# msyriac/orphics

Hardware: AMD Instinct MI355X
Metric: QE kappa reconstructions/sec on 8192^2 maps (higher is better)
Workload: dtype f64

## Files before the change

### include/orphics_amd.h

```cpp
#ifndef ORPHICS_AMD_H
#define ORPHICS_AMD_H

#include <stddef.h>
#include <stdint.h>

#ifdef __cplusplus
extern "C" {
#endif

#define OA_F32 0
#define OA_F64 1

typedef struct oa_plan oa_plan;

const char* oa_last_error(void);
#define OA_ABI_VERSION 416
int oa_version(void);
int oa_device_count(void);

int oa_plan_create(int ny, int nx, int dtype, oa_plan** out);
int oa_plan_destroy(oa_plan* p);
long oa_plan_kpitch(const oa_plan* p);
long oa_plan_scratch_bytes(const oa_plan* p);
int oa_plan_set_laxes(oa_plan* p, const double* host_ly, const double* host_lx);
// ... 13 lines not shown
int oa_qe_map_legs_cols(oa_plan* p, const void* real_map, const void* FG, const void* FH, void* gx, void* gy, void* h,
                        int width, int rband, void* stream);
int oa_qe_cols_div(oa_plan* p, const void* px_rows, const void* py_rows, const void* Fnorm, void* out, int accumulate,
                   int width, int rband, void* stream);

int oa_plan_set_filters(oa_plan* p, const void* FG, const void* FH, const void* Fnorm, int leg_cols, int kappa_cols,
                        int leg_rows, int kappa_rows, int mrow);
int oa_plan_set_col_grid(oa_plan* p, int mcol);
int oa_plan_col_grid(const oa_plan* p);
int oa_plan_band_grid(const oa_plan* p, int* my, int* mx);
int oa_qe_band_bind(oa_plan* p, int nfilters, const void* const* host_filters, int nnorms, const void* const* host_Fnorm, int leg_cols,
                    int kappa_cols, int leg_rows, int kappa_rows, int mrow, int mcol, int max_leg_planes);
int oa_qe_band_grid(const oa_plan* p, int* my, int* mx);
int oa_plan_rsplit(const oa_plan* p);
int oa_plan_div_fused(const oa_plan* p);
enum { OA_OPT_MC_BATCH = 1, OA_OPT_MV_BATCH = 2, OA_OPT_MV_ROWBATCH = 3, OA_OPT_MV_CHAIN = 4, OA_OPT_DIV_BIN = 5, OA_OPT_WIN_FUSED = 6, OA_OPT_DRAW_FUSED = 7 };
int oa_plan_set_option(oa_plan* p, int option, int value);
int oa_plan_set_bins(oa_plan* p, const int32_t* ids_hc, int nids, double norm, void* stream);
void* oa_plan_kappa(oa_plan* p);
const int64_t* oa_plan_bin_counts(oa_plan* p);
int oa_qe_tt(oa_plan* p, const void* real_map, const void* kX, const void* kY, void* out_kappa_hc, int zero_outside,
             void* stream);
int oa_qe_pol(oa_plan* p, int npieces, const double* host_signs, const void* const* host_FG, const void* const* host_FH,
              const int* host_swap, const void* kX, const void* kY, const void* Fnorm, void* out, int accumulate,
              int leg_cols, int kappa_cols, int leg_rows, int kappa_rows, int mrow, int zero_outside, void* stream);
int oa_qe_mv(oa_plan* p, int nest, const int* host_npieces, const double* host_signs, const void* const* host_FG,
             const void* const* host_FH, const int* host_swap, const void* const* host_kX, const void* const* host_kY,
             const void* const* host_Fnorm, void* out, int accumulate, int leg_cols, int kappa_cols, int leg_rows, int kappa_rows,
             int mrow, int zero_outside, void* stream);
int oa_qe_mv_maps(oa_plan* p, int nmaps, const void* const* host_maps, const void* rot_c, const void* rot_s, int nest,
                  const int* host_npieces, const double* host_signs, const void* const* host_FG, const void* const* host_FH,
// ... 135 lines not shown
```

### orphics_amd/csrc/common.hpp

```cpp
#pragma once
#include <hip/hip_runtime.h>
#include <cstdio>
#include <cstring>
#include <string>
#include "../../include/orphics_amd.h"
#include "cx.hpp"

namespace oa {

std::string& last_error_ref();

inline int fail(const std::string& msg) {
    last_error_ref() = msg;
    return 1;
}

#define OA_HIP(expr)                                                                              \
    do {                                                                                          \
        hipError_t _e = (expr);                                                                   \
        if (_e != hipSuccess)                                                                     \
            return ::oa::fail(std::string(#expr) + ": " + hipGetErrorString(_e) + " (" + __FILE__ + \
                              ":" + std::to_string(__LINE__) + ")");                              \
    } while (0)

// ... 49 lines not shown
    double* ly64;
    double* lx64;
    bool have_laxes;
    bool pow2;
    oa_plan* inner;
    int My, Mx;
    void* chirp_y; void* chirp_x;
    void* cz_bhat; void* cz_a; void* cz_f;
    void* cz_full;
    bool mixed;
    void* mr_twx; void* mr_twxh; void* mr_twy;
    void* pipe;
    void* rq8c[5];
    void* tw_y_small[16];
    void* tw_y_m3[16];
};

namespace oa {
int plan_ensure_scratch(oa_plan* p, size_t bytes);
int czt_setup(oa_plan* p);
void czt_release(oa_plan* p);
int czt_c2c(oa_plan* p, const void* in, void* out, int inverse, double scale, hipStream_t st);
int czt_r2c(oa_plan* p, const void* real_in, void* hc_out, double scale, hipStream_t st);
int czt_c2r(oa_plan* p, const void* hc_in, void* real_out, double scale, hipStream_t st);
bool mixed_sides_ok(int ny, int nx);
int mixed_setup(oa_plan* p);
void mixed_release(oa_plan* p);
int mixed_c2c(oa_plan* p, const void* in, void* out, int inverse, double scale, hipStream_t st);
int mixed_r2c(oa_plan* p, const void* real_in, void* hc_out, double scale, hipStream_t st);
int mixed_c2r(oa_plan* p, const void* hc_in, void* real_out, double scale, hipStream_t st);
// ... 105 lines not shown
```

### orphics_amd/csrc/fft.hip

```cpp
#include <algorithm>
#include <cmath>
#include <vector>
#include "fft_launch.hpp"
#include "fft_r2c_w64.hpp"
#include "fft_r2c_rs4096.hpp"
#include "fft_divbin.hpp"

namespace oa {

template <typename T, int MODE, class SEQ>
__global__ __launch_bounds__(row_maxnt<SEQ>(), waves_per_eu<T>()) void row_fft_kernel(RowArgs<T> a) {
    GpuCtx c{oa_dyn_smem};
    row_fft_body<T, MODE, SEQ>(c, a);
}

#ifndef OA_W64_OCC
#define OA_W64_OCC 1
#endif
__global__ __launch_bounds__(64, OA_W64_OCC) void row_r2c_w64_kernel(RowW64Args a) {
    GpuCtx c{oa_dyn_smem};
    row_r2c_w64_body(c, a);
}

template <typename T, class SEQ, int LR, bool PF>
// ... 33 lines not shown
__global__ __launch_bounds__((sizeof(T) == 8 ? 512 : 1024)) void col_fband_pack_kernel(ColFBandArgs<T> a, cx<T>* out) {
    GpuCtx c{nullptr};
    col_fband_pack_body<T, SEQF, LR, LOGC>(c, a, out);
}
template <typename T, class SEQF, int LR, int LOGC>
__global__ __launch_bounds__((sizeof(T) == 8 ? 512 : 1024), (sizeof(T) == 8 ? 2 : 4)) void col_fband_kernel(ColFBandArgs<T> a) {
    GpuCtx c{oa_dyn_smem};
    col_fband_body<T, SEQF, LR, LOGC>(c, a);
}

template <typename T, class SEQF, int LOGC>
__global__ __launch_bounds__((sizeof(T) == 8 ? 512 : 1024)) void col_fband3_pack_kernel(ColFBandArgs<T> a, cx<T>* out) {
    GpuCtx c{nullptr};
    col_fband3_pack_body<T, SEQF, LOGC>(c, a, out);
}
template <typename T, class SEQF, int LOGC>
__global__ __launch_bounds__((sizeof(T) == 8 ? 512 : 1024), (sizeof(T) == 8 ? 2 : 4)) void col_fband3_kernel(ColFBandArgs<T> a) {
    GpuCtx c{oa_dyn_smem};
    col_fband3_body<T, SEQF, LOGC>(c, a);
}

__global__ __launch_bounds__(128, 1) void row_r2c_w64x2_kernel(RowW64Args a) {
    GpuCtx c{oa_dyn_smem};
    row_r2c_w64x2_body(c, a);
}

#ifndef OA_QE_WAVES_PER_EU
#define OA_QE_WAVES_PER_EU 3
#endif
template <typename T, class SEQ> constexpr int qe_waves_per_eu() {
    return sizeof(T) == 8 ? 1 : (row_maxnt<SEQ>() > 256 ? 2 : OA_QE_WAVES_PER_EU);
}

template <typename T, class SEQ, int NZ>
// ... 274 lines not shown
    void col_fband_pack(int gx, int gy, int logMy, const ColFBandArgs<T>& a, cx<T>* out) {
        if (rc) return;
        const int lt = Fft2dPlan<T>::fband_lt(), nt = (1 << lt) / EPT;
        const bool narrow = lt < (sizeof(T) == 4 ? 14 : 13);
        const bool ok = dispatch_fband<T>(gy, logMy, narrow, [&](auto seq, auto lrc, auto lcc) {
            hipLaunchKernelGGL((col_fband_pack_kernel<T, decltype(seq), decltype(lrc)::value, decltype(lcc)::value>), dim3(gx, gy), dim3(nt), 0, st, a, out);
            const hipError_t e = hipGetLastError();
            if (e != hipSuccess) rc = fail(std::string("fft launch: ") + hipGetErrorString(e));
        });
        if (!ok) rc = fail("fft: unsupported R-split column stage");
    }
    template <typename T>
    void col_fband3(int gx, int gz, size_t smem, int logMy, const ColFBandArgs<T>& a) {
        if (rc) return;
        constexpr int nt = sizeof(T) == 4 ? 1024 : 512, lc11 = sizeof(T) == 4 ? 3 : 2;
        if (logMy == 11) go(col_fband3_kernel<T, Seq<16, 16, 8>, lc11>, dim3(gx, 4, gz), nt, smem, a);
        else if (logMy == 10) go(col_fband3_kernel<T, Seq<16, 8, 8>, lc11 + 1>, dim3(gx, 4, gz), nt, smem, a);
        else rc = fail("fft: unsupported 3 x 2^k R-split column stage");
    }
    template <typename T>
    void col_fband3_pack(int gx, int logMy, const ColFBandArgs<T>& a, cx<T>* out) {
        if (rc) return;
        constexpr int nt = sizeof(T) == 4 ? 1024 : 512, lc11 = sizeof(T) == 4 ? 3 : 2;
        if (logMy == 11) hipLaunchKernelGGL((col_fband3_pack_kernel<T, Seq<16, 16, 8>, lc11>), dim3(gx, 4), dim3(nt), 0, st, a, out);
        else if (logMy == 10) hipLaunchKernelGGL((col_fband3_pack_kernel<T, Seq<16, 8, 8>, lc11 + 1>), dim3(gx, 4), dim3(nt), 0, st, a, out);
        else { rc = fail("fft: unsupported 3 x 2^k R-split column stage"); return; }
        const hipError_t e = hipGetLastError();
        if (e != hipSuccess) rc = fail(std::string("fft launch: ") + hipGetErrorString(e));
    }
    template <typename T>
    void row_qe(int grid, int nt, size_t smem, const RowQeArgs<T>& a) {
        const bool ok = dispatch_seq_qe(a.logL, [&](auto seq) {
            using S = decltype(seq);
// ... 329 lines not shown
    const size_t plane = (size_t)p->ny * p->kp * sizeof(cx<T>);
    if (int rc = plan_ensure_scratch(p, 2 * plane)) return rc;
    HipLauncher q{st};
    auto f = view<T>(p);
    cx<T>* tA = (cx<T>*)p->scratch;
    cx<T>* tB = tA + (size_t)p->ny * p->kp;
    const int w = f.clampw(width);
    const long pw = pwork > 0 ? pwork : p->kp;
    if (lr > 0) {
        const auto cv = coarse_view<T>(p, my);
        if (is_m3(my)) {
            const int myf = m3_pow2(my);
            const long kplane3 = (long)myf * pw;
            if (stages & 1) f.rows_rsplit(q, map, tA, pw, kplane3, w, myf);
            if (stages & 4) f.legs_fband3(q, cv, (const cx<T>*)p->tw_y_small[ilog2(myf)], tA, kplane3, pw, (const T*)FG, (const T*)FH, (const T*)p->lxd,
                                          (const T*)p->lyd, (cx<T>*)gx, (cx<T>*)gy, (cx<T>*)h, width, rband, pout > 0 ? pout : p->kp, 1, 0, 0, (const cx<T>*)fgh);
            return q.rc;
        }
        const long kplane = (long)my * pw;
        if (stages & 1) f.rows_rsplit(q, map, tA, pw, kplane, w, my);
        if (stages & 4) f.legs_fband(q, cv, tA, kplane, pw, (const T*)FG, (const T*)FH, (const T*)p->lxd, (const T*)p->lyd, (cx<T>*)gx, (cx<T>*)gy,
                                     (cx<T>*)h, width, rband, pout > 0 ? pout : p->kp, 1, 0, 0, (const cx<T>*)fgh);
        return q.rc;
    }
    if (stages & 1) f.rows(q, ROW_R2C, map, p->nx / 2, tA, pw, (T)1, w);
    if (my > 0 && my < p->ny) {
        if (stages & 2) f.cols(q, tA, pw, tB, pw, w, false, (T)1, 1);
        if (stages & 4) {
            static const bool nofuse = exp_env("OA_NO_FWDLEGS_CG") != nullptr;
            const auto cv = coarse_view<T>(p, my);
            if (nofuse || !f.legs_cols_from_pass1_cg(q, cv, tB, (const T*)FG, (const T*)FH, (const T*)p->lxd, (const T*)p->lyd,
// ... 66 lines not shown
    const long ms = (long)p->ny * pl, cms = (long)my * pl, gms = (long)my * pk;
    if (2 * ms > (long)p->ny * p->kp || 2 * gms > (long)p->ny * p->kp) return -1;
    const size_t plane = (size_t)p->ny * p->kp * sizeof(cx<T>);
    if (int rc = plan_ensure_scratch(p, 2 * plane)) return rc;
    HipLauncher q{st};
    q.fuse = fuse;
    cx<T>* tA = (cx<T>*)p->scratch;
    cx<T>* tB = tA + (size_t)p->ny * p->kp;
    const double s = 1.0 / ((double)p->ny * p->nx), sy = (double)p->ny / my;
    if (lr) {
        const int myf = m3 ? m3_pow2(my) : my;
        const long kplane = (long)myf * pl;
        f.rows_rsplit(q, map0, tA, pl, kplane, wi, myf);
        f.rows_rsplit(q, map1, tA + ms, pl, kplane, wi, myf);
        if (m3) f.legs_fband3(q, cv, (const cx<T>*)p->tw_y_small[ilog2(myf)], tA, kplane, pl, (const T*)FG, (const T*)FH, (const T*)p->lxd, (const T*)p->lyd,
                              (cx<T>*)c0, (cx<T>*)c1, (cx<T>*)c2, wl, rl, pl, 2, ms, cms, (const cx<T>*)fgh);
        else
        f.legs_fband(q, cv, tA, kplane, pl, (const T*)FG, (const T*)FH, (const T*)p->lxd, (const T*)p->lyd, (cx<T>*)c0, (cx<T>*)c1, (cx<T>*)c2, wl, rl,
                     pl, 2, ms, cms, (const cx<T>*)fgh);
        cv.rows_qe(q, (const cx<T>*)c0, (const cx<T>*)c1, (const cx<T>*)c2, (cx<T>*)g0, (cx<T>*)g1, (T)(s * s * sy), 0, wi, wo, mrow, pl, pk, 2, cms, gms,
                   -1, nullptr, lr);
        if (m3) cv.cols_div3(q, (const cx<T>*)g0, (const cx<T>*)g1, (const T*)Fn, (const T*)p->lxd, (const T*)p->lyd, (cx<T>*)out0, 0, wk, rk, pk, 2, gms,
                             (long)((cx<T>*)out1 - (cx<T>*)out0));
        else
        cv.cols_div(q, (const cx<T>*)g0, (const cx<T>*)g1, (const T*)Fn, (const T*)p->lxd, (const T*)p->lyd, (cx<T>*)out0, tA, tB, 0, wk, rk, pk, 2,
                    gms, gms, (long)((cx<T>*)out1 - (cx<T>*)out0));
        return q.rc;
    }
    f.rows(q, ROW_R2C, map0, p->nx / 2, tA, pl, (T)1, wi);
    f.rows(q, ROW_R2C, map1, p->nx / 2, tA + ms, pl, (T)1, wi);
    const cx<T>* ins[2] = {tA, tA + ms};
// ... 419 lines not shown
```

### orphics_amd/csrc/fft_fband.hpp

```cpp
#pragma once
#include "fft_kernels.hpp"
#include "fft_mixed.hpp"
#ifndef FB_STAMP
#define FB_STAMP(i)
#endif

namespace oa {

template <typename T>
struct ColFBandArgs {
    const cx<T>* in;
    long kplane, pitch;
    const T* FG; const T* FH;
    long fpitch;
    const cx<T>* fgh;
    const T* lxd; const T* lyd;
    cx<T>* gx; cx<T>* gy; cx<T>* h;
    long opitch;
    int width;
    const cx<T>* tw;
    int ny_full, rband;
    long in_moff, out_moff;
    const cx<T>* tw3 = nullptr;
};

template <typename T>
struct FBandStore2 {
    cx<T>* base;
    unsigned kstride;
    int ncols;
    const cx<T>* twl;
    int h, k1;
    template <typename U> OA_HD void put(int k, int c, cx<U> v) const {
        if (c >= ncols) return;
        if (k1) v = v * tw_lds(twl, h, k);
        base[(unsigned)k * kstride + (unsigned)c] = swp(v);
    }
};
// ... 158 lines not shown
    template <typename U> OA_HD void put(int k, int c, cx<U> v) const {
        if (c >= ncols) return;
        const int y = 3 * k + q;
        base[(unsigned)y * kstride + (unsigned)c] = swp(v * ti[y]);
    }
};

template <int Q>
OA_HD int fband3_bin(int m, int e) {
    constexpr int Ns = 2 * Q, RL = 8;
    if (e == 0) return m;
    if (e == 2) return m + Q + (RL - 1) * Ns;
    return 2 * m >= Q ? m + (RL - 1) * Ns : m + Q;
}

template <typename T, class SEQF, int LOGC, class Ctx>
OA_HD void col_fband3_body(Ctx& ctx, const ColFBandArgs<T>& a) {
    cx<T>* s = reinterpret_cast<cx<T>*>(ctx.smem());
    constexpr int logL = seq_total_log<SEQF>();
    constexpr int R = 4;
    constexpr int RL = SEQF::get(SEQF::n - 1), NB = EPT / RL;
    static_assert(RL == 8 && NB == 2, "col_fband3: the last forward radix is 8");
    constexpr int logQ = logL - 4, Q = 1 << logQ, Mq = 3 * Q;
    constexpr int C = 1 << LOGC;
    constexpr int NT = (1 << (logL + LOGC)) / EPT;
    constexpr int NTS = (Q << LOGC) / EPT;
    const int tid = ctx.tid();
    int tile = ctx.bid_x();
    if ((sizeof(cx<T>) << LOGC) < 128) {
        constexpr int G = 128 / (int)(sizeof(cx<T>) << LOGC), GW = 8 * G;
        const int nt = ctx.grid_x(), base = tile & ~(GW - 1), r = tile & (GW - 1);
        if (base + GW <= nt) tile = base + G * (r & 7) + (r >> 3);
    }
    const int c0 = tile << LOGC;
    const int k1 = ctx.bid_y();
    int ncols = a.width - c0;
    if (ncols > C) ncols = C;
    cx<T> gv[EPT];
    cx<T>* twl = s + (1 << (logL + LOGC));
    cx<T>* twq = twl + tw_lds_size(logL);
    cx<T>* ti = twq + tw_lds_size(logQ);
    FB_STAMP(0);
    tw_lds_fill<T>(ctx, twl, a.tw, logL, logL, NT);
    tw_lds_fill<T>(ctx, twq, a.tw, logL, logQ, NT);
    for (int i = tid; i < Mq; i += NT) ti[i] = a.tw3[(unsigned)k1 * (unsigned)i];
    ctx.sync();
    FB_STAMP(1);
    const long zmap = ctx.bid_z();
    const int c = tid & (C - 1), m = tid >> LOGC;
    const bool ok = c < ncols;
    T fgv[3], fhv[3], lyv[3];
    bool lv[3];
    const cx<T>* fq = a.fgh ? a.fgh + (((long)k1 * ctx.grid_x() + tile) * 3) * NT + tid : nullptr;
    const T lx = ldg(a.lxd + (ok ? c0 + c : 0));
    const cx<T> wq1 = ldg(a.tw3 + 4 * m), wq2 = ldg(a.tw3 + 8 * m);
#pragma unroll
    for (int e = 0; e < 3; ++e) {
        const int yf = k1 + R * fband3_bin<Q>(m, e);
        bool live = ok;
        if (a.rband) live = ok && !(yf >= a.rband && yf <= a.ny_full - a.rband);
        if (fq) {
            const cx<T> f = ldg(fq + e * NT);
            fgv[e] = f.x; fhv[e] = f.y;
        } else {
            const long fi = live ? (long)yf * a.fpitch + (c0 + c) : 0;
            fgv[e] = ldg(a.FG + fi);
            fhv[e] = ldg(a.FH + fi);
        }
        lyv[e] = ldg(a.lyd + (live ? yf : 0));
        lv[e] = live;
    }
    FB_STAMP(2);
    const ColLoad<T> ld{a.in + zmap * a.in_moff + (long)k1 * a.kplane + c0, (unsigned)a.pitch, ncols, false};
    col_pipeline_to_regs<T, SEQF>(ctx, s, gv, tid, NT, LOGC, twl, logL, ld);
    ctx.sync();
    FB_STAMP(3);
    cx<T> zh[3], zx[3], zy[3];
    const cx<T> xm = (2 * m >= Q) ? gv[RL - 1] : gv[RL];
#pragma unroll
    for (int e = 0; e < 3; ++e) {
        const cx<T> x = e == 0 ? gv[0] : (e == 2 ? gv[2 * RL - 1] : xm);
        const T fg = lv[e] ? fgv[e] : (T)0, fh = lv[e] ? fhv[e] : (T)0, ly = lv[e] ? lyv[e] : (T)0;
        const cx<T> g = mul_pi(x * fg);
        zh[e] = swp(x * fh);
        zx[e] = swp(g * (ok ? lx : (T)0));
        zy[e] = swp(g * ly);
    }
    MrDft<T, 3>::run(zh); MrDft<T, 3>::run(zx); MrDft<T, 3>::run(zy);
#pragma unroll
    for (int q = 0; q < 3; ++q) {
        const int at = ((q * Q + m) << LOGC) + c;
        cx<T> h = zh[q], x = zx[q], y = zy[q];
        if (q == 1) { h = h * wq1; x = x * wq1; y = y * wq1; }
        if (q == 2) { h = h * wq2; x = x * wq2; y = y * wq2; }
        s[at] = h;
        s[(Mq << LOGC) + at] = x;
        s[2 * (Mq << LOGC) + at] = y;
    }
    ctx.sync();
    FB_STAMP(4);
    const int sid = tid / NTS, tq = tid - sid * NTS;
    const int leg = sid / 3, q = sid - 3 * leg;
    cx<T>* outp = leg == 0 ? a.h : (leg == 1 ? a.gx : a.gy);
    using SI = typename SeqOf<logQ>::type;
    const FBand3Store<T> st{outp + zmap * a.out_moff + (long)k1 * a.opitch + c0, (unsigned)(R * a.opitch), leg < 3 ? ncols : 0, ti, q};
    fft_pipeline<T, false, false, true, SI>(ctx, s + sid * (Q << LOGC), tq, NTS, logQ, LOGC, 0, twq, logQ, NoLoad{}, st);
    FB_STAMP(5);
}

template <typename T, class SEQF, int LOGC, class Ctx>
OA_HD void col_fband3_pack_body(Ctx& ctx, const ColFBandArgs<T>& a, cx<T>* out) {
    constexpr int logL = seq_total_log<SEQF>(), R = 4, Q = 1 << (logL - 4), C = 1 << LOGC;
    constexpr int NT = (1 << (logL + LOGC)) / EPT;
    const int tid = ctx.tid(), tile = ctx.bid_x(), k1 = ctx.bid_y(), c0 = tile << LOGC;
    const int c = tid & (C - 1), m = tid >> LOGC;
    cx<T>* o = out + (((long)k1 * ctx.grid_x() + tile) * 3) * NT + tid;
#pragma unroll
    for (int e = 0; e < 3; ++e) {
        const int yf = k1 + R * fband3_bin<Q>(m, e);
        bool live = c0 + c < a.width;
        if (a.rband) live = live && !(yf >= a.rband && yf <= a.ny_full - a.rband);
        cx<T> f = mk<T>((T)0, (T)0);
// ... 7 lines not shown
```

### orphics_amd/csrc/fft_plan.hpp

```cpp
#pragma once
#include <cmath>
#include <cstdlib>
#include <vector>
#include "fft_kernels.hpp"
#include "fft_fband.hpp"
#include "fft_rowqe8.hpp"

namespace oa {

template <typename T>
inline std::vector<cx<T>> make_twiddles(int M) {
    std::vector<cx<T>> t((size_t)M);
    const long double tau = 6.283185307179586476925286766559005768L;
    for (int k = 0; k < M; ++k) {
        long double a = tau * (long double)k / (long double)M;
        t[(size_t)k].x = (T)cosl(a);
        t[(size_t)k].y = (T)(-sinl(a));
    }
    return t;
}

inline long kpitch_for(int nx) { return nx / 2 + 16; }

inline bool is_pow2(int v) { return v > 0 && (v & (v - 1)) == 0; }
inline bool is_m3(int v) { return v >= 3 && v % 3 == 0 && is_pow2(v / 3); }
inline int m3_pow2(int v) { return v / 3 * 4; }

template <typename T>
struct Fft2dPlan {
    int ny = 0, nx = 0, logNy = 0, logNx = 0;
    long kp = 0;
    const cx<T>* tw_x = nullptr;
    const cx<T>* tw_y = nullptr;
    const cx<T>* rq8c[RQ8_NGRIDS] = {};
    bool rq8_ready(int m) const { const int i = rq8_slot(m); return rowqe8_on() && i >= 0 && rq8c[i] != nullptr; }
    int ny_full = 0;
    int yshift() const { return ny_full > ny ? ny_full - ny : 0; }
    static constexpr int COLC = COL_LOGC;

    long work_pitch(int w) const {
        const long c = 1L << COLC;
// ... 67 lines not shown
        a.in = Y; a.kplane = kplane; a.pitch = pin; a.FG = FG; a.FH = FH; a.fpitch = kp; a.lxd = lxd; a.lyd = lyd; a.fgh = fgh;
        a.gx = gx; a.gy = gy; a.h = h; a.opitch = pout; a.width = clampw(wmax); a.tw = cv.tw_y; a.ny_full = ny; a.rband = clampr(rband);
        a.in_moff = in_moff; a.out_moff = out_moff;
        const int lt = fband_lt(), lc = lt - cv.logNy, Cs = 1 << lc;
        const int logMq = cv.logNy - (logNy - cv.logNy);
        const size_t smem = ((size_t)(1 << lt) + tw_lds_size(cv.logNy) + tw_lds_size(logMq) + (logNy - cv.logNy == 1 ? 0 : (1 << logMq))) * sizeof(cx<T>);
        if (pack_out) q.col_fband_pack((a.width + Cs - 1) / Cs, 1 << (logNy - cv.logNy), cv.logNy, a, pack_out);
        else q.col_fband((a.width + Cs - 1) / Cs, 1 << (logNy - cv.logNy), nmaps, smem, cv.logNy, a);
    }
    static bool has_rsplit3(int logNy, int logNx, int my3, int wl) {
        if (!is_m3(my3)) return false;
        const int myf = m3_pow2(my3);
        return (myf == 1024 || myf == 2048) && logNy - ilog2(myf) == 2 && has_rsplit(logNy, logNx, myf, wl) && fband_lt() == (sizeof(T) == 4 ? 14 : 13) &&
               div_lt() == fband_lt();
    }
    template <class Launcher>
    void legs_fband3(Launcher& q, const Fft2dPlan<T>& cv, const cx<T>* twf, const cx<T>* Y, long kplane, long pin, const T* FG, const T* FH,
                     const T* lxd, const T* lyd, cx<T>* gx, cx<T>* gy, cx<T>* h, int wmax, int rband, long pout, int nmaps = 1, long in_moff = 0,
                     long out_moff = 0, const cx<T>* fgh = nullptr, cx<T>* pack_out = nullptr) const {
        ColFBandArgs<T> a{};
        a.in = Y; a.kplane = kplane; a.pitch = pin; a.FG = FG; a.FH = FH; a.fpitch = kp; a.lxd = lxd; a.lyd = lyd; a.fgh = fgh;
        a.gx = gx; a.gy = gy; a.h = h; a.opitch = pout; a.width = clampw(wmax); a.tw = twf; a.tw3 = cv.tw_y; a.ny_full = ny; a.rband = clampr(rband);
        a.in_moff = in_moff; a.out_moff = out_moff;
        const int logMy = logNy - 2, lt = fband_lt(), lc = lt - logMy, Cs = 1 << lc, logQ = logMy - 4;
        const size_t smem = ((size_t)(1 << lt) + tw_lds_size(logMy) + tw_lds_size(logQ) + 3 * (1 << logQ)) * sizeof(cx<T>);
        if (pack_out) q.col_fband3_pack((a.width + Cs - 1) / Cs, logMy, a, pack_out);
        else q.col_fband3((a.width + Cs - 1) / Cs, nmaps, smem, logMy, a);
    }
    long fband_table_entries(const Fft2dPlan<T>& cv, int wmax) const {
        const int lc = fband_lt() - cv.logNy, Cs = 1 << lc;
        return (long)((clampw(wmax) + Cs - 1) / Cs) * Cs * cv.ny;
    }
    long fband3_table_entries(const Fft2dPlan<T>& cv, int wmax) const {
        const int lc = fband_lt() - (logNy - 2), Cs = 1 << lc;
        return (long)((clampw(wmax) + Cs - 1) / Cs) * Cs * cv.ny;
    }

    double row_grid_scale(int mrow) const { return (mrow > 0 && mrow < nx) ? (double)nx / (double)mrow : 1.0; }
    bool rows_qe_is_pair(int win, int wout, int mrow) const {
        if (mrow <= 0 || ny % 2) return false;
// ... 343 lines not shown
```

### orphics_amd/csrc/pipeline.hip

```cpp
#include <dlfcn.h>
#include <cstdlib>
#include <algorithm>
#include <functional>
#include <string>
#include <utility>
#include <vector>
#include "common.hpp"
#include "fft_plan.hpp"
#include "divbin_runs.hpp"

namespace oa {

constexpr int MC_BATCH_MAX = 6;

struct DevBuf {
    void* p = nullptr;
    size_t bytes = 0;
    int reserve(size_t need, bool zero = false) {
        if (bytes >= need) return 0;
        if (p) { OA_HIP(hipDeviceSynchronize()); release(); }
        OA_HIP(hipMalloc(&p, need));
        bytes = need;
        if (zero) OA_HIP(hipMemset(p, 0, need));
        return 0;
// ... 52 lines not shown
    DivTabs& tabs_of(int rows) { return (my3 && rows == my3) ? dt[1] : dt[0]; }
    const DivTabs& tabs_of(int rows) const { return (my3 && rows == my3) ? dt[1] : dt[0]; }
    unsigned long bind_gen = 1;
    DevBuf fb_t;
    unsigned long fb_gen = 0;
    int fb_my = 0, fb_wl = 0, fb_rl = 0;
    void** mv_ftab = nullptr;
    std::vector<const void*> mv_fkey;
    int opt_mc_batch = MC_BATCH_MAX;
    bool opt_mv_batch = true;
    bool opt_mv_rowbatch = true;
    bool opt_mv_chain = true;
    bool opt_divbin = true;
    bool opt_win_fused = true;
    bool opt_win_fused_set = false;
    int opt_draw_fused = -1;
    oa_plan* band = nullptr;
    int bmy = 0, bmx = 0;
    DevBuf bplanes;
    DevBuf bids;
    DevBuf brows;
    DevBuf bwin;
    DevBuf bsplit;
    int bs_cap = 0;
    DevBuf bs_tab;
    std::vector<const void*> bs_key;
    struct PolBind {
        bool bound = false;
        unsigned long gen = 0;
        oa_plan* plan = nullptr;
// ... 188 lines not shown

int oa_plan_set_option(oa_plan* p, int option, int value) {
    OA_REQUIRE(p, "oa_plan_set_option: NULL plan");
    Pipeline* q = pipe_of(p);
    switch (option) {
        case OA_OPT_MC_BATCH:
            OA_REQUIRE(value >= 0 && value <= MC_BATCH_MAX, "oa_plan_set_option: OA_OPT_MC_BATCH takes 0 (default) .. 6");
            q->opt_mc_batch = value ? value : MC_BATCH_MAX; return 0;
        case OA_OPT_MV_BATCH: q->opt_mv_batch = value != 0; return 0;
        case OA_OPT_MV_ROWBATCH: q->opt_mv_rowbatch = value != 0; return 0;
        case OA_OPT_MV_CHAIN: q->opt_mv_chain = value != 0; return 0;
        case OA_OPT_DIV_BIN: q->opt_divbin = value != 0; return 0;
        case OA_OPT_WIN_FUSED:
            q->opt_win_fused = value != 0; q->opt_win_fused_set = value >= 0; return 0;
        case OA_OPT_DRAW_FUSED: q->opt_draw_fused = value < 0 ? -1 : (value != 0); return 0;
        default: return fail("oa_plan_set_option: unknown option");
    }
}
}
namespace oa {
static void band_options(Pipeline* q) {
    for (oa_plan* inner : {q->band, q->pb.plan}) {
        if (!inner || !inner->pipe) continue;
        Pipeline* b = (Pipeline*)inner->pipe;
        b->opt_mc_batch = q->opt_mc_batch; b->opt_mv_batch = q->opt_mv_batch; b->opt_mv_rowbatch = q->opt_mv_rowbatch;
        b->opt_mv_chain = q->opt_mv_chain; b->opt_divbin = q->opt_divbin; b->opt_win_fused = q->opt_win_fused;
    }
}
}
extern "C" {
int oa_plan_rdn0_batched(const oa_plan* p) { return (p && p->pipe) ? ((const Pipeline*)p->pipe)->rdn0_ran_batched : 0; }
int oa_plan_rsplit(const oa_plan* p) {
    if (!p || !p->pipe) return 0;
    const Pipeline* q = (const Pipeline*)p->pipe;
    return q->FG ? (1 << qe_rsplit_lr(p, q->map_grid(), q->wl, q->wk, q->mrow)) & ~1 : 0;
}

int oa_plan_div_fused(const oa_plan* p) {
    if (!p || !p->pipe) return 0;
    const Pipeline* q = (const Pipeline*)p->pipe;
    if (p->mixed) { band_options((Pipeline*)q); return (q->FG && q->ids && q->band) ? oa_plan_div_fused(q->band) : 0; }
// ... 2171 lines not shown
```

### orphics_amd/engine.py

```python
import ctypes

import numpy as np
import torch

from . import _lib
from ._lib import OA_F32, OA_F64, check


def _ptr(t):
    return ctypes.c_void_p(t.data_ptr()) if t is not None else None


def _stream():
    return ctypes.c_void_p(torch.cuda.current_stream().cuda_stream)


def _dirty(t):
    mark_dirty(t)
    return t


_RDT = {"f32": torch.float32, "f64": torch.float64}
_CDT = {"f32": torch.complex64, "f64": torch.complex128}
_CODE = {"f32": OA_F32, "f64": OA_F64}
# ... 399 lines not shown
        n = self._same(a, b)
        if a.dtype != self.rdt or b.dtype != self.rdt:
            raise ValueError("axpby: dtype mismatch")
        out = torch.empty_like(a) if out is None else self._out(out, a, self.rdt, "axpby")
        check(self.lib.oa_axpby_real(self.code, _ptr(a), _ptr(b), _ptr(out), float(alpha), float(beta), n, _stream()))
        return out

    def rot2(self, c, s, i1, i2):
        n = self._same(c, s, i1, i2)
        if c.dtype != self.rdt or i1.dtype != self.cdt or i2.dtype != self.cdt or s.dtype != self.rdt:
            raise ValueError("rot2: dtype mismatch")
        o1, o2 = torch.empty_like(i1), torch.empty_like(i2)
        check(self.lib.oa_rot2(self.code, _ptr(c), _ptr(s), _ptr(i1), _ptr(i2), _ptr(o1), _ptr(o2), n, _stream()))
        return o1, o2

    OPTIONS = {"mc_batch": 1, "mv_batch": 2, "mv_rowbatch": 3, "mv_chain": 4, "div_bin": 5, "win_fused": 6, "draw_fused": 7}

    def set_option(self, name, value):
        if name not in self.OPTIONS:
            raise ValueError("unknown plan option %r (one of %s)" % (name, sorted(self.OPTIONS)))
        check(self.lib.oa_plan_set_option(self.plan, self.OPTIONS[name], int(value)))
        self._options = dict(getattr(self, "_options", {}), **{name: int(value)})

    def copy_options_to(self, other):
        for name, value in getattr(self, "_options", {}).items():
            other.set_option(name, value)

    def band_grid(self, leg_cols, kappa_cols, leg_rows, kappa_rows, mrow=-1, mcol=-1):
        if not self.mixed:
            return None
        return band_grid(self.ny, self.nx, leg_cols, kappa_cols, leg_rows, kappa_rows, mrow, mcol)
# ... 273 lines not shown
```

Baseline: 6074.

## Process multiple k-planes per workgroup in fband3 column kernel with prefetch

Templates the 3x2^k R-split column-band kernel on KPW, so one workgroup handles 1, 2 or 4 of the four residue planes in a loop. Twiddle tables are loaded once per workgroup, and the next plane's input taps and filters are prefetched while the current plane's FFT stages run. This amortizes setup and hides global-load latency, at the cost of fewer workgroups, more registers and more LDS for twiddles. The default KPW is 2 only for f32 with at least two maps, so this f64 workload keeps KPW=1 and runs only the restructured single-plane body.

```diff
diff --git a/include/orphics_amd.h b/include/orphics_amd.h
--- a/include/orphics_amd.h
+++ b/include/orphics_amd.h
@@ -51,7 +51,8 @@
 int oa_qe_band_grid(const oa_plan* p, int* my, int* mx);
 int oa_plan_rsplit(const oa_plan* p);
 int oa_plan_div_fused(const oa_plan* p);
-enum { OA_OPT_MC_BATCH = 1, OA_OPT_MV_BATCH = 2, OA_OPT_MV_ROWBATCH = 3, OA_OPT_MV_CHAIN = 4, OA_OPT_DIV_BIN = 5, OA_OPT_WIN_FUSED = 6, OA_OPT_DRAW_FUSED = 7 };
+enum { OA_OPT_MC_BATCH = 1, OA_OPT_MV_BATCH = 2, OA_OPT_MV_ROWBATCH = 3, OA_OPT_MV_CHAIN = 4, OA_OPT_DIV_BIN = 5, OA_OPT_WIN_FUSED = 6, OA_OPT_DRAW_FUSED = 7,
+       OA_OPT_FBAND3_KPW = 8 };
 int oa_plan_set_option(oa_plan* p, int option, int value);
 int oa_plan_set_bins(oa_plan* p, const int32_t* ids_hc, int nids, double norm, void* stream);
 void* oa_plan_kappa(oa_plan* p);
diff --git a/orphics_amd/csrc/common.hpp b/orphics_amd/csrc/common.hpp
--- a/orphics_amd/csrc/common.hpp
+++ b/orphics_amd/csrc/common.hpp
@@ -87,6 +87,7 @@
     void* rq8c[5];
     void* tw_y_small[16];
     void* tw_y_m3[16];
+    int fband3_kpw;
 };
 
 namespace oa {
diff --git a/orphics_amd/csrc/fft.hip b/orphics_amd/csrc/fft.hip
--- a/orphics_amd/csrc/fft.hip
+++ b/orphics_amd/csrc/fft.hip
@@ -71,10 +71,10 @@
     GpuCtx c{nullptr};
     col_fband3_pack_body<T, SEQF, LOGC>(c, a, out);
 }
-template <typename T, class SEQF, int LOGC>
+template <typename T, class SEQF, int LOGC, int KPW>
 __global__ __launch_bounds__((sizeof(T) == 8 ? 512 : 1024), (sizeof(T) == 8 ? 2 : 4)) void col_fband3_kernel(ColFBandArgs<T> a) {
     GpuCtx c{oa_dyn_smem};
-    col_fband3_body<T, SEQF, LOGC>(c, a);
+    col_fband3_body<T, SEQF, LOGC, KPW>(c, a);
 }
 
 __global__ __launch_bounds__(128, 1) void row_r2c_w64x2_kernel(RowW64Args a) {
@@ -379,9 +379,16 @@
     void col_fband3(int gx, int gz, size_t smem, int logMy, const ColFBandArgs<T>& a) {
         if (rc) return;
         constexpr int nt = sizeof(T) == 4 ? 1024 : 512, lc11 = sizeof(T) == 4 ? 3 : 2;
-        if (logMy == 11) go(col_fband3_kernel<T, Seq<16, 16, 8>, lc11>, dim3(gx, 4, gz), nt, smem, a);
-        else if (logMy == 10) go(col_fband3_kernel<T, Seq<16, 8, 8>, lc11 + 1>, dim3(gx, 4, gz), nt, smem, a);
-        else rc = fail("fft: unsupported 3 x 2^k R-split column stage");
+        auto launch = [&](auto kc) {
+            constexpr int KPW = decltype(kc)::value;
+            if (logMy == 11) go(col_fband3_kernel<T, Seq<16, 16, 8>, lc11, KPW>, dim3(gx, 4 / KPW, gz), nt, smem, a);
+            else if (logMy == 10) go(col_fband3_kernel<T, Seq<16, 8, 8>, lc11 + 1, KPW>, dim3(gx, 4 / KPW, gz), nt, smem, a);
+            else rc = fail("fft: unsupported 3 x 2^k R-split column stage");
+        };
+        if (a.kpw == 1) launch(std::integral_constant<int, 1>{});
+        else if (a.kpw == 2 || (a.kpw == 4 && sizeof(T) == 4)) launch(std::integral_constant<int, 2>{});
+        else if (a.kpw == 4) { if constexpr (sizeof(T) == 8) launch(std::integral_constant<int, 4>{}); }
+        else rc = fail("fft: the 3 x 2^k R-split column stage takes 1, 2 or 4 planes per workgroup");
     }
     template <typename T>
     void col_fband3_pack(int gx, int logMy, const ColFBandArgs<T>& a, cx<T>* out) {
@@ -741,7 +748,8 @@
             const long kplane3 = (long)myf * pw;
             if (stages & 1) f.rows_rsplit(q, map, tA, pw, kplane3, w, myf);
             if (stages & 4) f.legs_fband3(q, cv, (const cx<T>*)p->tw_y_small[ilog2(myf)], tA, kplane3, pw, (const T*)FG, (const T*)FH, (const T*)p->lxd,
-                                          (const T*)p->lyd, (cx<T>*)gx, (cx<T>*)gy, (cx<T>*)h, width, rband, pout > 0 ? pout : p->kp, 1, 0, 0, (const cx<T>*)fgh);
+                                          (const T*)p->lyd, (cx<T>*)gx, (cx<T>*)gy, (cx<T>*)h, width, rband, pout > 0 ? pout : p->kp, 1, 0, 0, (const cx<T>*)fgh, nullptr,
+                                          p->fband3_kpw);
             return q.rc;
         }
         const long kplane = (long)my * pw;
@@ -838,7 +846,7 @@
         f.rows_rsplit(q, map0, tA, pl, kplane, wi, myf);
         f.rows_rsplit(q, map1, tA + ms, pl, kplane, wi, myf);
         if (m3) f.legs_fband3(q, cv, (const cx<T>*)p->tw_y_small[ilog2(myf)], tA, kplane, pl, (const T*)FG, (const T*)FH, (const T*)p->lxd, (const T*)p->lyd,
-                              (cx<T>*)c0, (cx<T>*)c1, (cx<T>*)c2, wl, rl, pl, 2, ms, cms, (const cx<T>*)fgh);
+                              (cx<T>*)c0, (cx<T>*)c1, (cx<T>*)c2, wl, rl, pl, 2, ms, cms, (const cx<T>*)fgh, nullptr, p->fband3_kpw);
         else
         f.legs_fband(q, cv, tA, kplane, pl, (const T*)FG, (const T*)FH, (const T*)p->lxd, (const T*)p->lyd, (cx<T>*)c0, (cx<T>*)c1, (cx<T>*)c2, wl, rl,
                      pl, 2, ms, cms, (const cx<T>*)fgh);
diff --git a/orphics_amd/csrc/fft_fband.hpp b/orphics_amd/csrc/fft_fband.hpp
--- a/orphics_amd/csrc/fft_fband.hpp
+++ b/orphics_amd/csrc/fft_fband.hpp
@@ -22,6 +22,7 @@
     int ny_full, rband;
     long in_moff, out_moff;
     const cx<T>* tw3 = nullptr;
+    int kpw = 1;
 };
 
 template <typename T>
@@ -210,18 +211,28 @@
     return 2 * m >= Q ? m + (RL - 1) * Ns : m + Q;
 }
 
-template <typename T, class SEQF, int LOGC, class Ctx>
+template <typename T>
+struct FBand3Plane {
+    cx<T> tap[EPT];
+    T fg[3], fh[3], ly[3];
+    bool lv[3];
+};
+
+template <typename T, class SEQF, int LOGC, int KPW = 1, class Ctx>
 OA_HD void col_fband3_body(Ctx& ctx, const ColFBandArgs<T>& a) {
     cx<T>* s = reinterpret_cast<cx<T>*>(ctx.smem());
     constexpr int logL = seq_total_log<SEQF>();
-    constexpr int R = 4;
-    constexpr int RL = SEQF::get(SEQF::n - 1), NB = EPT / RL;
+    constexpr int R = 4, KS = R / KPW;
+    static_assert(KPW == 1 || KPW == 2 || KPW == 4, "col_fband3: 1, 2 or 4 planes per workgroup");
+    constexpr int R0 = SEQF::get(0), RL = SEQF::get(SEQF::n - 1), NB = EPT / RL;
+    static_assert(SEQF::n == 3 && R0 == EPT, "col_fband3: three forward stages, the first one butterfly of EPT points per thread");
     static_assert(RL == 8 && NB == 2, "col_fband3: the last forward radix is 8");
     constexpr int logQ = logL - 4, Q = 1 << logQ, Mq = 3 * Q;
     constexpr int C = 1 << LOGC;
     constexpr int NT = (1 << (logL + LOGC)) / EPT;
     constexpr int NTS = (Q << LOGC) / EPT;
-    const int tid = ctx.tid();
+    constexpr int l0 = Log2x<SEQF::r0>::v, l1 = l0 + Log2x<SEQF::r1>::v;
+    const int tid0 = ctx.tid();
     int tile = ctx.bid_x();
     if ((sizeof(cx<T>) << LOGC) < 128) {
         constexpr int G = 128 / (int)(sizeof(cx<T>) << LOGC), GW = 8 * G;
@@ -229,79 +240,109 @@
         if (base + GW <= nt) tile = base + G * (r & 7) + (r >> 3);
     }
     const int c0 = tile << LOGC;
-    const int k1 = ctx.bid_y();
+    const int k10 = ctx.bid_y();
     int ncols = a.width - c0;
     if (ncols > C) ncols = C;
-    cx<T> gv[EPT];
     cx<T>* twl = s + (1 << (logL + LOGC));
     cx<T>* twq = twl + tw_lds_size(logL);
     cx<T>* ti = twq + tw_lds_size(logQ);
+    const long zmap = ctx.bid_z();
     FB_STAMP(0);
+    auto request = [&](int k1, int tid, FBand3Plane<T>& pl) {
+        const int c = tid & (C - 1), m = tid >> LOGC;
+        const bool ok = c < ncols;
+        const ColLoad<T> ld{a.in + zmap * a.in_moff + (long)k1 * a.kplane + c0, (unsigned)a.pitch, ncols, false};
+#pragma unroll
+        for (int t = 0; t < R0; ++t) pl.tap[t] = ld.template get<T>(m + (t << (logL - l0)), c);
+        const cx<T>* fq = a.fgh ? a.fgh + (((long)k1 * ctx.grid_x() + tile) * 3) * NT + tid : nullptr;
+#pragma unroll
+        for (int e = 0; e < 3; ++e) {
+            const int yf = k1 + R * fband3_bin<Q>(m, e);
+            bool live = ok;
+            if (a.rband) live = ok && !(yf >= a.rband && yf <= a.ny_full - a.rband);
+            if (fq) {
+                const cx<T> f = ldg(fq + e * NT);
+                pl.fg[e] = f.x; pl.fh[e] = f.y;
+            } else {
+                const long fi = live ? (long)yf * a.fpitch + (c0 + c) : 0;
+                pl.fg[e] = ldg(a.FG + fi);
+                pl.fh[e] = ldg(a.FH + fi);
+            }
+            pl.ly[e] = ldg(a.lyd + (live ? yf : 0));
+            pl.lv[e] = live;
+        }
+    };
+    FBand3Plane<T> cur, nxt;
+    request(k10, tid0, cur);
+    const T lx = ldg(a.lxd + ((tid0 & (C - 1)) < ncols ? c0 + (tid0 & (C - 1)) : 0));
+    const cx<T> wq1 = ldg(a.tw3 + 4 * (tid0 >> LOGC)), wq2 = ldg(a.tw3 + 8 * (tid0 >> LOGC));
+    FB_STAMP(1);
     tw_lds_fill<T>(ctx, twl, a.tw, logL, logL, NT);
     tw_lds_fill<T>(ctx, twq, a.tw, logL, logQ, NT);
-    for (int i = tid; i < Mq; i += NT) ti[i] = a.tw3[(unsigned)k1 * (unsigned)i];
-    ctx.sync();
-    FB_STAMP(1);
-    const long zmap = ctx.bid_z();
-    const int c = tid & (C - 1), m = tid >> LOGC;
-    const bool ok = c < ncols;
-    T fgv[3], fhv[3], lyv[3];
-    bool lv[3];
-    const cx<T>* fq = a.fgh ? a.fgh + (((long)k1 * ctx.grid_x() + tile) * 3) * NT + tid : nullptr;
-    const T lx = ldg(a.lxd + (ok ? c0 + c : 0));
-    const cx<T> wq1 = ldg(a.tw3 + 4 * m), wq2 = ldg(a.tw3 + 8 * m);
-#pragma unroll
-    for (int e = 0; e < 3; ++e) {
-        const int yf = k1 + R * fband3_bin<Q>(m, e);
-        bool live = ok;
-        if (a.rband) live = ok && !(yf >= a.rband && yf <= a.ny_full - a.rband);
-        if (fq) {
-            const cx<T> f = ldg(fq + e * NT);
-            fgv[e] = f.x; fhv[e] = f.y;
-        } else {
-            const long fi = live ? (long)yf * a.fpitch + (c0 + c) : 0;
-            fgv[e] = ldg(a.FG + fi);
-            fhv[e] = ldg(a.FH + fi);
-        }
-        lyv[e] = ldg(a.lyd + (live ? yf : 0));
-        lv[e] = live;
-    }
+#pragma unroll
+    for (int i = 0; i < KPW; ++i)
+        for (int y = tid0; y < Mq; y += NT) ti[i * Mq + y] = a.tw3[(unsigned)(k10 + i * KS) * (unsigned)y];
     FB_STAMP(2);
-    const ColLoad<T> ld{a.in + zmap * a.in_moff + (long)k1 * a.kplane + c0, (unsigned)a.pitch, ncols, false};
-    col_pipeline_to_regs<T, SEQF>(ctx, s, gv, tid, NT, LOGC, twl, logL, ld);
-    ctx.sync();
-    FB_STAMP(3);
-    cx<T> zh[3], zx[3], zy[3];
-    const cx<T> xm = (2 * m >= Q) ? gv[RL - 1] : gv[RL];
-#pragma unroll
-    for (int e = 0; e < 3; ++e) {
-        const cx<T> x = e == 0 ? gv[0] : (e == 2 ? gv[2 * RL - 1] : xm);
-        const T fg = lv[e] ? fgv[e] : (T)0, fh = lv[e] ? fhv[e] : (T)0, ly = lv[e] ? lyv[e] : (T)0;
-        const cx<T> g = mul_pi(x * fg);
-        zh[e] = swp(x * fh);
-        zx[e] = swp(g * (ok ? lx : (T)0));
-        zy[e] = swp(g * ly);
-    }
-    MrDft<T, 3>::run(zh); MrDft<T, 3>::run(zx); MrDft<T, 3>::run(zy);
-#pragma unroll
-    for (int q = 0; q < 3; ++q) {
-        const int at = ((q * Q + m) << LOGC) + c;
-        cx<T> h = zh[q], x = zx[q], y = zy[q];
-        if (q == 1) { h = h * wq1; x = x * wq1; y = y * wq1; }
-        if (q == 2) { h = h * wq2; x = x * wq2; y = y * wq2; }
-        s[at] = h;
-        s[(Mq << LOGC) + at] = x;
-        s[2 * (Mq << LOGC) + at] = y;
-    }
-    ctx.sync();
-    FB_STAMP(4);
-    const int sid = tid / NTS, tq = tid - sid * NTS;
-    const int leg = sid / 3, q = sid - 3 * leg;
-    cx<T>* outp = leg == 0 ? a.h : (leg == 1 ? a.gx : a.gy);
     using SI = typename SeqOf<logQ>::type;
-    const FBand3Store<T> st{outp + zmap * a.out_moff + (long)k1 * a.opitch + c0, (unsigned)(R * a.opitch), leg < 3 ? ncols : 0, ti, q};
-    fft_pipeline<T, false, false, true, SI>(ctx, s + sid * (Q << LOGC), tq, NTS, logQ, LOGC, 0, twq, logQ, NoLoad{}, st);
-    FB_STAMP(5);
+#pragma unroll
+    for (int i = 0; i < KPW; ++i) {
+        const int k1 = k10 + i * KS;
+        int tid = tid0;
+#if defined(__HIP_DEVICE_COMPILE__)
+        if constexpr (KPW > 1) asm volatile("" : "+v"(tid));
+#endif
+        const int c = tid & (C - 1), m = tid >> LOGC;
+        const bool ok = c < ncols;
+        const int sid = tid / NTS, tq = tid - sid * NTS;
+        const int leg = sid / 3, q = sid - 3 * leg;
+        cx<T>* outp = leg == 0 ? a.h : (leg == 1 ? a.gx : a.gy);
+        cx<T> gv[EPT];
+        Dft<T, R0>::run(cur.tap);
+        stage_out<T, R0, false, false>(s, cur.tap, tid, NT, logL, LOGC, 0, 0, NoStore{});
+        T fgv[3], fhv[3], lyv[3];
+        bool lv[3];
+#pragma unroll
+        for (int e = 0; e < 3; ++e) { fgv[e] = cur.fg[e]; fhv[e] = cur.fh[e]; lyv[e] = cur.ly[e]; lv[e] = cur.lv[e]; }
+        ctx.sync();
+        if (sizeof(T) == 8 && i + 1 < KPW) request(k1 + KS, tid, nxt);
+        stage<T, SEQF::r1, false, false, false>(ctx, s, tid, NT, logL, LOGC, 0, l0, twl, logL, NoLoad{}, NoStore{});
+        ctx.sync();
+        if (sizeof(T) == 4 && i + 1 < KPW) request(k1 + KS, tid, nxt);
+        stage_in<T, RL, false, false>(s, gv, tid, NT, logL, LOGC, 0, l1, twl, logL, NoLoad{});
+        ctx.sync();
+        FB_STAMP(3);
+        cx<T> zh[3], zx[3], zy[3];
+        const cx<T> xm = (2 * m >= Q) ? gv[RL - 1] : gv[RL];
+#pragma unroll
+        for (int e = 0; e < 3; ++e) {
+            const cx<T> x = e == 0 ? gv[0] : (e == 2 ? gv[2 * RL - 1] : xm);
+            const T fg = lv[e] ? fgv[e] : (T)0, fh = lv[e] ? fhv[e] : (T)0, ly = lv[e] ? lyv[e] : (T)0;
+            const cx<T> g = mul_pi(x * fg);
+            zh[e] = swp(x * fh);
+            zx[e] = swp(g * (ok ? lx : (T)0));
+            zy[e] = swp(g * ly);
+        }
+        MrDft<T, 3>::run(zh); MrDft<T, 3>::run(zx); MrDft<T, 3>::run(zy);
+#pragma unroll
+        for (int r = 0; r < 3; ++r) {
+            const int at = ((r * Q + m) << LOGC) + c;
+            cx<T> h = zh[r], x = zx[r], y = zy[r];
+            if (r == 1) { h = h * wq1; x = x * wq1; y = y * wq1; }
+            if (r == 2) { h = h * wq2; x = x * wq2; y = y * wq2; }
+            s[at] = h;
+            s[(Mq << LOGC) + at] = x;
+            s[2 * (Mq << LOGC) + at] = y;
+        }
+        ctx.sync();
+        FB_STAMP(4);
+        const FBand3Store<T> st{outp + zmap * a.out_moff + (long)k1 * a.opitch + c0, (unsigned)(R * a.opitch), leg < 3 ? ncols : 0, ti + i * Mq, q};
+        fft_pipeline<T, false, false, true, SI>(ctx, s + sid * (Q << LOGC), tq, NTS, logQ, LOGC, 0, twq, logQ, NoLoad{}, st);
+        FB_STAMP(5);
+        if (i + 1 < KPW) {
+            ctx.sync();
+            cur = nxt;
+        }
+    }
 }
 
 template <typename T, class SEQF, int LOGC, class Ctx>
diff --git a/orphics_amd/csrc/fft_plan.hpp b/orphics_amd/csrc/fft_plan.hpp
--- a/orphics_amd/csrc/fft_plan.hpp
+++ b/orphics_amd/csrc/fft_plan.hpp
@@ -25,6 +25,7 @@
 inline bool is_pow2(int v) { return v > 0 && (v & (v - 1)) == 0; }
 inline bool is_m3(int v) { return v >= 3 && v % 3 == 0 && is_pow2(v / 3); }
 inline int m3_pow2(int v) { return v / 3 * 4; }
+inline int fband3_kpw_default(bool f64, int nmaps) { return (!f64 && nmaps >= 2) ? 2 : 1; }
 
 template <typename T>
 struct Fft2dPlan {
@@ -122,16 +123,22 @@
         return (myf == 1024 || myf == 2048) && logNy - ilog2(myf) == 2 && has_rsplit(logNy, logNx, myf, wl) && fband_lt() == (sizeof(T) == 4 ? 14 : 13) &&
                div_lt() == fband_lt();
     }
+    static int fband3_kpw(int nmaps) {
+        static const int forced = [] { const char* e = exp_env("OA_FBAND3_KPW"); return e ? atoi(e) : 0; }();
+        if (forced == 1 || forced == 2 || forced == 4) return forced;
+        return fband3_kpw_default(sizeof(T) == 8, nmaps);
+    }
     template <class Launcher>
     void legs_fband3(Launcher& q, const Fft2dPlan<T>& cv, const cx<T>* twf, const cx<T>* Y, long kplane, long pin, const T* FG, const T* FH,
                      const T* lxd, const T* lyd, cx<T>* gx, cx<T>* gy, cx<T>* h, int wmax, int rband, long pout, int nmaps = 1, long in_moff = 0,
-                     long out_moff = 0, const cx<T>* fgh = nullptr, cx<T>* pack_out = nullptr) const {
+                     long out_moff = 0, const cx<T>* fgh = nullptr, cx<T>* pack_out = nullptr, int kpw = 0) const {
         ColFBandArgs<T> a{};
         a.in = Y; a.kplane = kplane; a.pitch = pin; a.FG = FG; a.FH = FH; a.fpitch = kp; a.lxd = lxd; a.lyd = lyd; a.fgh = fgh;
         a.gx = gx; a.gy = gy; a.h = h; a.opitch = pout; a.width = clampw(wmax); a.tw = twf; a.tw3 = cv.tw_y; a.ny_full = ny; a.rband = clampr(rband);
         a.in_moff = in_moff; a.out_moff = out_moff;
+        a.kpw = (kpw == 1 || kpw == 2 || kpw == 4) ? kpw : fband3_kpw(nmaps);
         const int logMy = logNy - 2, lt = fband_lt(), lc = lt - logMy, Cs = 1 << lc, logQ = logMy - 4;
-        const size_t smem = ((size_t)(1 << lt) + tw_lds_size(logMy) + tw_lds_size(logQ) + 3 * (1 << logQ)) * sizeof(cx<T>);
+        const size_t smem = ((size_t)(1 << lt) + tw_lds_size(logMy) + tw_lds_size(logQ) + a.kpw * 3 * (1 << logQ)) * sizeof(cx<T>);
         if (pack_out) q.col_fband3_pack((a.width + Cs - 1) / Cs, logMy, a, pack_out);
         else q.col_fband3((a.width + Cs - 1) / Cs, nmaps, smem, logMy, a);
     }
diff --git a/orphics_amd/csrc/pipeline.hip b/orphics_amd/csrc/pipeline.hip
--- a/orphics_amd/csrc/pipeline.hip
+++ b/orphics_amd/csrc/pipeline.hip
@@ -90,6 +90,7 @@
     bool opt_divbin = true;
     bool opt_win_fused = true;
     bool opt_win_fused_set = false;
+    int opt_fband3_kpw = 0;
     int opt_draw_fused = -1;
     oa_plan* band = nullptr;
     int bmy = 0, bmx = 0;
@@ -308,6 +309,9 @@
         case OA_OPT_WIN_FUSED:
             q->opt_win_fused = value != 0; q->opt_win_fused_set = value >= 0; return 0;
         case OA_OPT_DRAW_FUSED: q->opt_draw_fused = value < 0 ? -1 : (value != 0); return 0;
+        case OA_OPT_FBAND3_KPW:
+            OA_REQUIRE(value == 0 || value == 1 || value == 2 || value == 4, "oa_plan_set_option: OA_OPT_FBAND3_KPW takes 0 (default), 1, 2 or 4");
+            q->opt_fband3_kpw = p->fband3_kpw = value; return 0;
         default: return fail("oa_plan_set_option: unknown option");
     }
 }
@@ -319,6 +323,7 @@
         Pipeline* b = (Pipeline*)inner->pipe;
         b->opt_mc_batch = q->opt_mc_batch; b->opt_mv_batch = q->opt_mv_batch; b->opt_mv_rowbatch = q->opt_mv_rowbatch;
         b->opt_mv_chain = q->opt_mv_chain; b->opt_divbin = q->opt_divbin; b->opt_win_fused = q->opt_win_fused;
+        b->opt_fband3_kpw = inner->fband3_kpw = q->opt_fband3_kpw;
     }
 }
 }
diff --git a/orphics_amd/engine.py b/orphics_amd/engine.py
--- a/orphics_amd/engine.py
+++ b/orphics_amd/engine.py
@@ -437,7 +437,8 @@
         check(self.lib.oa_rot2(self.code, _ptr(c), _ptr(s), _ptr(i1), _ptr(i2), _ptr(o1), _ptr(o2), n, _stream()))
         return o1, o2
 
-    OPTIONS = {"mc_batch": 1, "mv_batch": 2, "mv_rowbatch": 3, "mv_chain": 4, "div_bin": 5, "win_fused": 6, "draw_fused": 7}
+    OPTIONS = {"mc_batch": 1, "mv_batch": 2, "mv_rowbatch": 3, "mv_chain": 4, "div_bin": 5, "win_fused": 6, "draw_fused": 7,
+               "fband3_kpw": 8}
 
     def set_option(self, name, value):
         if name not in self.OPTIONS:
```

Result: slower. 5975 (-1.6%).
